# Jiawei-Yang/Denoising-ViT

Measured on AMD Instinct MI355X. Metric: stage-1 images denoised/sec (DINOv2-B/14, 518px, 1k Adam steps), higher is better.
Workload: dtype bf16

## Files before the change

denoising-vit_amd/csrc/dvt_vit.hip:

```cpp
#include <math.h>

#include <type_traits>

#include "../../include/dvt_vit.h"
#include "dvt_common.h"
#include "dvt_ln_row.h"

typedef short bf16x8 __attribute__((ext_vector_type(8)));
typedef short bf16x4 __attribute__((ext_vector_type(4)));
typedef float f32x4 __attribute__((ext_vector_type(4)));
typedef unsigned short bf16_t;

extern int g_f32x3_exact_attention, g_f32x3_unfused;

namespace {

typedef __bf16 hw_bf16x2 __attribute__((ext_vector_type(2)));
typedef float f32x2 __attribute__((ext_vector_type(2)));

__device__ __forceinline__ uint32_t pack2(float a, float b) {
  const hw_bf16x2 v = __builtin_convertvector((f32x2){a, b}, hw_bf16x2);
  return __builtin_bit_cast(uint32_t, v);
}
__device__ __forceinline__ bf16_t f2bf(float f) { return (bf16_t)(pack2(f, 0.f) & 0xffffu); }
// ... 261 lines not shown
        for (int rp = 0; rp < 2; ++rp) {
          const float mine0 = v[rp], mine1 = v[rp + 2];
          const float send = odd ? mine0 : mine1;
          const float recv = __shfl_xor(send, 1, 64);
          const int r = odd ? rp + 2 : rp;
          const uint32_t w = odd ? pack2(recv, mine1) : pack2(mine0, recv);
          const int ncol = odd ? n - 1 : n;
          *reinterpret_cast<uint32_t*>(p.out + (size_t)(mrow + r) * ldo + ncol) = w;
        }
      }
    }
  }
}

template <int EPI>
__global__ __launch_bounds__(256) void gemm_bf16_kernel(GemmBArgs p) {
  __shared__ __attribute__((aligned(16))) char smem[2 * STAGE_BYTES];
  const int tid = threadIdx.x, lane = tid & 63, wave = tid >> 6;
  const int wm = wave >> 1, wn = wave & 1;
  const TileMap tm = map_tile(blockIdx.x, gridDim.x, p.M / GBM, p.N / GBN, p.group);
  const int m0 = tm.m * GBM, n0 = tm.n * GBN;

  f32x4 acc[4][4];
#pragma unroll
  for (int i = 0; i < 4; ++i)
#pragma unroll
    for (int j = 0; j < 4; ++j) acc[i][j] = (f32x4){0.f, 0.f, 0.f, 0.f};

  const int nk = p.K / GBK;
  stage_tile(p.A, p.K, m0, 0, smem, wave, lane);
  stage_tile(p.W, p.K, n0, 0, smem + GBM * GBK * 2, wave, lane);
  __syncthreads();
  for (int kt = 0; kt < nk; ++kt) {
    char* cur = smem + (kt & 1) * STAGE_BYTES;
    char* nxt = smem + ((kt + 1) & 1) * STAGE_BYTES;
    if (kt + 1 < nk) {
      stage_tile(p.A, p.K, m0, (kt + 1) * GBK, nxt, wave, lane);
      stage_tile(p.W, p.K, n0, (kt + 1) * GBK, nxt + GBM * GBK * 2, wave, lane);
    }
    const char* As = cur;
    const char* Bs = cur + GBM * GBK * 2;
#pragma unroll
    for (int ks = 0; ks < 2; ++ks) {
      bf16x8 a[4], b[4];
      const int chunk = ks * 4 + (lane >> 4);
#pragma unroll
      for (int i = 0; i < 4; ++i) a[i] = read_frag(As, wm * 64 + i * 16 + (lane & 15), chunk);
#pragma unroll
      for (int j = 0; j < 4; ++j) b[j] = read_frag(Bs, wn * 64 + j * 16 + (lane & 15), chunk);
#pragma unroll
      for (int i = 0; i < 4; ++i)
#pragma unroll
        for (int j = 0; j < 4; ++j)
          acc[i][j] = __builtin_amdgcn_mfma_f32_16x16x32_bf16(a[i], b[j], acc[i][j], 0, 0, 0);
    }
    __syncthreads();
  }

  gemm_epilogue<EPI>(p, acc, m0, n0, wm, wn, lane);
}

constexpr int EP_LD = 68;
constexpr int EP_WAVE_BYTES = 64 * EP_LD * 4;

template <int NI>
__device__ __forceinline__ void ln_fold(const GemmBArgs& p, f32x4 (&acc)[NI][4], int mrow0, int ncol0, int lane);

struct NextTilePf {
  const bf16_t* src;
  int n;
  unsigned d0, d1;
};
__device__ __forceinline__ void pf_issue(NextTilePf& f) {
  if (f.src == nullptr) return;
  asm volatile("global_load_dword %0, %1, off" : "=v"(f.d0) : "v"(f.src) : "memory");
  if (f.n > 1) asm volatile("global_load_dword %0, %1, off offset:128" : "=v"(f.d1) : "v"(f.src) : "memory");
}
__device__ __forceinline__ void pf_retire(NextTilePf& f) {
  if (f.src == nullptr) return;
  asm volatile("s_waitcnt vmcnt(0)" ::: "memory");
  asm volatile("" ::"v"(f.d0), "v"(f.d1));
}

template <int EPI, int NI = 4>
__device__ __forceinline__ void gemm_epilogue_lds(const GemmBArgs& p, f32x4 (&acc)[NI][4], int m0,
                                                  int n0, int wm, int wn, int wave, int lane,
                                                  char* smem, char* blk0 = nullptr, NextTilePf* pf = nullptr) {
  static_assert(NI == 4 || NI == 2, "64- or 32-row passes");
  constexpr int ROWS = NI * 16;
  const int g = lane >> 4, lc = lane & 15;
  const bool ln = (IS_QKV(EPI) || IS_GELU(EPI) || EPI == EPI_SWIGLU) && p.ln_stats != nullptr;
  float* blk = reinterpret_cast<float*>(blk0 != nullptr ? blk0 : smem + wave * EP_WAVE_BYTES);
  const int nb = n0 + wn * 64;
  if (IS_QKV(EPI) && n0 >= 2 * p.dim) {
    const int mbv = m0 + wm * 64;
    constexpr int TCH = ROWS / 8, FPP = 64 / TCH, NPASS = 64 / FPP;
    const int tc = lane & (TCH - 1), dl = lane / TCH;
    float4 stq[4];
    float csd[NPASS], bfd[NPASS];
    if (ln) {
      const float4* sp = reinterpret_cast<const float4*>(p.ln_stats + mbv + tc * 8);
#pragma unroll
      for (int q = 0; q < 4; ++q) stq[q] = sp[q];
#pragma unroll
      for (int it = 0; it < NPASS; ++it) {
        csd[it] = p.ln_cs[nb + it * FPP + dl];
        bfd[it] = p.bias[nb + it * FPP + dl];
      }
    }
#pragma unroll
    for (int j = 0; j < 4; ++j) {
      const float bias = (p.bias != nullptr && !ln) ? p.bias[nb + j * 16 + lc] : 0.f;
#pragma unroll
      for (int i = 0; i < NI; ++i) {
        const float4 t4 = make_float4(acc[i][j][0] + bias, acc[i][j][1] + bias, acc[i][j][2] + bias, acc[i][j][3] + bias);
        *reinterpret_cast<float4*>(blk + (j * 16 + lc) * EP_LD + i * 16 + 4 * g) = t4;
      }
    }
    asm volatile("s_waitcnt lgkmcnt(0)" ::: "memory");
    const int f0 = nb - 2 * p.dim, hh = f0 >> 6;
    const int trow = mbv + tc * 8, bimg = trow / p.s_pad, s0 = trow - bimg * p.s_pad;
    const bool vst = trow < p.vt_rows;
    bf16_t* const vrow = p.vt + ((size_t)(bimg * p.heads + hh) * 64) * p.s_pad + s0;
#pragma unroll
    for (int it = 0; it < NPASS; ++it) {
      if (pf != nullptr && it == 1) pf_issue(*pf);
      const int d = it * FPP + dl;
      const float4 a = *reinterpret_cast<const float4*>(blk + d * EP_LD + tc * 8);
      const float4 b = *reinterpret_cast<const float4*>(blk + d * EP_LD + tc * 8 + 4);
      float v[8] = {a.x, a.y, a.z, a.w, b.x, b.y, b.z, b.w};
      if (ln) {
        const float cs = csd[it], bf = bfd[it];
#pragma unroll
        for (int q = 0; q < 4; ++q) {
          v[2 * q] = fmaf(stq[q].y, v[2 * q] - stq[q].x * cs, bf);
          v[2 * q + 1] = fmaf(stq[q].w, v[2 * q + 1] - stq[q].z * cs, bf);
        }
      }
      typedef unsigned u32x4v_t __attribute__((ext_vector_type(4)));
      const u32x4v_t hi = {pack2(v[0], v[1]), pack2(v[2], v[3]), pack2(v[4], v[5]), pack2(v[6], v[7])};
      if (vst) *reinterpret_cast<u32x4v_t*>(vrow + (size_t)d * p.s_pad) = hi;
      if constexpr (EPI == EPI_QKV_X3) {
        u32x4v_t lo;
#pragma unroll
        for (int q = 0; q < 4; ++q)
          lo[q] = pack2(v[2 * q] - __uint_as_float(hi[q] << 16), v[2 * q + 1] - __uint_as_float(hi[q] & 0xffff0000u));
        if (vst) *reinterpret_cast<u32x4v_t*>(p.vt_lo + (vrow - p.vt) + (size_t)d * p.s_pad) = lo;
      }
    }
    return;
  }
  float2 st_row = make_float2(0.f, 0.f);
  if (ln && lane < ROWS) st_row = p.ln_stats[m0 + wm * 64 + lane];
  const int c8_ln = (lane & 7) * 8;
  float4 cs0 = make_float4(0.f, 0.f, 0.f, 0.f), cs1 = cs0, bf0 = cs0, bf1 = cs0;
  if (ln && EPI != EPI_RESID && EPI != EPI_EMBED && EPI != EPI_F32 && EPI != EPI_SWIGLU) {
    cs0 = *reinterpret_cast<const float4*>(p.ln_cs + nb + c8_ln);
    cs1 = *reinterpret_cast<const float4*>(p.ln_cs + nb + c8_ln + 4);
    bf0 = *reinterpret_cast<const float4*>(p.bias + nb + c8_ln);
    bf1 = *reinterpret_cast<const float4*>(p.bias + nb + c8_ln + 4);
  }
#ifdef DVT_LAB
  if (!(p.abl & 1))
#endif
#pragma unroll
  for (int j = 0; j < 4; ++j) {
    const float bias = (p.bias != nullptr && !ln) ? p.bias[nb + j * 16 + lc] : 0.f;
#pragma unroll
    for (int i = 0; i < NI; ++i)
#pragma unroll
      for (int r = 0; r < 4; ++r) blk[(i * 16 + 4 * g + r) * EP_LD + j * 16 + lc] = acc[i][j][r] + bias;
  }
  if (ln && lane < ROWS) *reinterpret_cast<float2*>(blk + lane * EP_LD + 64) = st_row;
  asm volatile("s_waitcnt lgkmcnt(0)" ::: "memory");
  const int mb = m0 + wm * 64;
  if constexpr (EPI == EPI_SWIGLU) {
    const int c8 = (lane & 3) * 8, ldo = p.N >> 1;
    const int rsub = ((lane >> 2) & 1) + 8 * ((lane >> 3) & 1) + 2 * (lane >> 4);
    alignas(16) float csg[8], csv[8], bfg[8], bfv[8];
    if (ln) {
#pragma unroll
      for (int q = 0; q < 8; q += 4) {
        *reinterpret_cast<float4*>(csg + q) = *reinterpret_cast<const float4*>(p.ln_cs + nb + c8 + q);
        *reinterpret_cast<float4*>(csv + q) = *reinterpret_cast<const float4*>(p.ln_cs + nb + 32 + c8 + q);
        *reinterpret_cast<float4*>(bfg + q) = *reinterpret_cast<const float4*>(p.bias + nb + c8 + q);
        *reinterpret_cast<float4*>(bfv + q) = *reinterpret_cast<const float4*>(p.bias + nb + 32 + c8 + q);
      }
    }
#pragma unroll 1
    for (int it = 0; it < ROWS / 16; ++it) {
      if (pf != nullptr && it == 1) pf_issue(*pf);
      const int row = it * 16 + rsub;
      alignas(16) float gt[8], vl[8];
#pragma unroll
      for (int q = 0; q < 8; q += 4) {
        *reinterpret_cast<float4*>(gt + q) = *reinterpret_cast<const float4*>(blk + row * EP_LD + c8 + q);
        *reinterpret_cast<float4*>(vl + q) = *reinterpret_cast<const float4*>(blk + row * EP_LD + 32 + c8 + q);
      }
      if (ln) {
        const float2 stv = *reinterpret_cast<const float2*>(blk + row * EP_LD + 64);
#pragma unroll
        for (int q = 0; q < 8; ++q) {
          gt[q] = fmaf(stv.y, gt[q] - stv.x * csg[q], bfg[q]);
          vl[q] = fmaf(stv.y, vl[q] - stv.x * csv[q], bfv[q]);
        }
      }
#pragma unroll
      for (int q = 0; q < 8; ++q) gt[q] = silu_log2(gt[q]) * vl[q];
      typedef unsigned u32x4s_t __attribute__((ext_vector_type(4)));
      const u32x4s_t val = {pack2(gt[0], gt[1]), pack2(gt[2], gt[3]), pack2(gt[4], gt[5]), pack2(gt[6], gt[7])};
      u32x4s_t* dst = reinterpret_cast<u32x4s_t*>(p.out + (size_t)(mb + row) * ldo + (nb >> 1) + c8);
      if (p.nt_store)
        __builtin_nontemporal_store(val, dst);
      else
        *dst = val;
    }
    return;
  }
  if (EPI == EPI_RESID || EPI == EPI_EMBED || EPI == EPI_F32) {
    const int c4 = lc * 4;
    float4 gm = make_float4(1.f, 1.f, 1.f, 1.f);
    if (EPI == EPI_RESID) gm = *reinterpret_cast<const float4*>(p.gamma + nb + c4);
#pragma unroll 4
    for (int it = 0; it < ROWS / 4; ++it) {
      const int row = it * 4 + g;
      if (pf != nullptr && it == ROWS / 8 && EPI == EPI_F32) pf_issue(*pf);
      const float4 v = *reinterpret_cast<const float4*>(blk + row * EP_LD + c4);
      const int t = mb + row;
      float4* px = reinterpret_cast<float4*>(p.x + (size_t)t * p.N + nb + c4);
      if (EPI == EPI_RESID) {
        float4 o = *px;
        o.x += gm.x * v.x;
        o.y += gm.y * v.y;
        o.z += gm.z * v.z;
        o.w += gm.w * v.w;
        *px = o;
      } else if (EPI == EPI_F32) {
        *px = v;
      } else {
        const int sidx = t % p.s_pad;
        float4 o = make_float4(0.f, 0.f, 0.f, 0.f);
        if (sidx < p.n_prefix) {
          o = *reinterpret_cast<const float4*>(p.cls + (size_t)sidx * p.N + nb + c4);
          if (p.pos_has_cls && sidx == 0) {
            const float4 q = *reinterpret_cast<const float4*>(p.pos + nb + c4);
            o = make_float4(o.x + q.x, o.y + q.y, o.z + q.z, o.w + q.w);
          }
        } else if (sidx < p.n_tokens) {
          const float4 q = *reinterpret_cast<const float4*>(
// ... 80 lines not shown
    for (int r = 0; r < 4; ++r) {
      const float2 st = p.ln_stats[mrow0 + i * 16 + 4 * g + r];
#pragma unroll
      for (int j = 0; j < 4; ++j) acc[i][j][r] = st.y * (acc[i][j][r] - st.x * cs[j]);
    }
}

__global__ __launch_bounds__(256) void ln_stats_finalize_kernel(const float2* __restrict__ part, int P, int M, float inv_n,
                                                                float eps, float2* __restrict__ stats) {
  const int m = blockIdx.x * 256 + threadIdx.x;
  if (m >= M) return;
  float s1 = 0.f, s2 = 0.f;
  for (int q = 0; q < P; ++q) {
    const float2 v = part[(size_t)q * M + m];
    s1 += v.x;
    s2 += v.y;
  }
  const float mu = s1 * inv_n;
  const float var = fmaxf(s2 * inv_n - mu * mu, 0.f);
  stats[m] = make_float2(mu, rsqrtf(var + eps));
}

template <int NV = 4>
__global__ __launch_bounds__(256) void ln_cast_stats_kernel(const float* __restrict__ x, bf16_t* __restrict__ xb,
                                                            float2* __restrict__ stats, int rows, int dim, float eps) {
  const int row = blockIdx.x * 4 + (threadIdx.x >> 6), lane = threadIdx.x & 63;
  if (row >= rows) return;
  const float4* xr = reinterpret_cast<const float4*>(x + (size_t)row * dim);
  const int nq = dim >> 2;
  float4 v[NV];
  float sum = 0.f;
#pragma unroll
  for (int i = 0; i < NV; ++i) {
    const int q = lane + 64 * i;
    if (q < nq) {
      v[i] = xr[q];
      sum += v[i].x + v[i].y + v[i].z + v[i].w;
      uint2 pk;
      pk.x = pack2(v[i].x, v[i].y);
      pk.y = pack2(v[i].z, v[i].w);
      reinterpret_cast<uint2*>(xb + (size_t)row * dim)[q] = pk;
    }
  }
  const float mean = wave_sum(sum) / (float)dim;
  float var = 0.f;
#pragma unroll
  for (int i = 0; i < NV; ++i) {
    const int q = lane + 64 * i;
    if (q < nq) {
      const float a = v[i].x - mean, b = v[i].y - mean, c = v[i].z - mean, d = v[i].w - mean;
      var += a * a + b * b + c * c + d * d;
    }
  }
  const float rstd = rsqrtf(wave_sum(var) / (float)dim + eps);
  if (lane == 0) stats[row] = make_float2(mean, rstd);
}

__global__ __launch_bounds__(256) void swiglu_act_kernel(const uint4* __restrict__ h, uint4* __restrict__ hid, long long n8,
                                                         int hq) {
  for (long long q = (long long)blockIdx.x * 256 + threadIdx.x; q < n8; q += (long long)gridDim.x * 256) {
    const long long r = q / hq;
    const int c = (int)(q - r * hq);
    const uint4 gv = h[r * 2 * hq + c], vv = h[r * 2 * hq + hq + c];
    const unsigned gw[4] = {gv.x, gv.y, gv.z, gv.w}, vw[4] = {vv.x, vv.y, vv.z, vv.w};
    unsigned o[4];
#pragma unroll
    for (int i = 0; i < 4; ++i) {
      const float g0 = __uint_as_float(gw[i] << 16), g1 = __uint_as_float(gw[i] & 0xffff0000u);
      const float v0 = __uint_as_float(vw[i] << 16), v1 = __uint_as_float(vw[i] & 0xffff0000u);
      o[i] = pack2(silu_log2(g0) * v0, silu_log2(g1) * v1);
    }
    hid[q] = make_uint4(o[0], o[1], o[2], o[3]);
  }
}

__device__ __forceinline__ float row16_sum(float v) {
  v += __builtin_bit_cast(float, __builtin_amdgcn_update_dpp(0, __builtin_bit_cast(int, v), 0x128, 0xf, 0xf, false));
  v += __builtin_bit_cast(float, __builtin_amdgcn_update_dpp(0, __builtin_bit_cast(int, v), 0x124, 0xf, 0xf, false));
  v += __builtin_bit_cast(float, __builtin_amdgcn_update_dpp(0, __builtin_bit_cast(int, v), 0x122, 0xf, 0xf, false));
  v += __builtin_bit_cast(float, __builtin_amdgcn_update_dpp(0, __builtin_bit_cast(int, v), 0x121, 0xf, 0xf, false));
  return v;
}

__device__ __forceinline__ void gemm_epilogue_resid_sq(const GemmBArgs& p, f32x4 (&acc)[8][4], int mb,
                                                       int nb, int wave, int lane, char* smem, NextTilePf* pf = nullptr) {
  const int g = lane >> 4, lc = lane & 15, c4 = lc * 4;
  float* blk = reinterpret_cast<float*>(smem + wave * EP_WAVE_BYTES);
  const __amdgpu_buffer_rsrc_t xr = __builtin_amdgcn_make_buffer_rsrc(
      p.x + (size_t)mb * p.N + nb, 0, 0x7fffffff, 0x00020000);
  const int loff = (g * p.N + c4) * 4;
  const int rstep = p.N * 16;
  typedef int i32x4_t __attribute__((ext_vector_type(4)));
#define RS_LD(it) __builtin_bit_cast(float4, __builtin_amdgcn_raw_buffer_load_b128(xr, loff, (it) * rstep, 0))
#define RS_ST(it, v) __builtin_amdgcn_raw_buffer_store_b128(__builtin_bit_cast(i32x4_t, v), xr, loff + (it) * rstep, 0, 0)
#define RS_LN(it, o)                                                                                    \
  do {                                                                                                  \
    const int row_ = mb + (it) * 4 + g;                                                                 \
    uint2 pk_;                                                                                          \
    pk_.x = pack2((o).x, (o).y);                                                                        \
    pk_.y = pack2((o).z, (o).w);                                                                        \
    *reinterpret_cast<uint2*>(p.xb + (size_t)row_ * p.N + nb + c4) = pk_;                               \
    float s1_ = ((o).x + (o).y) + ((o).z + (o).w);                                                      \
    float s2_ = ((o).x * (o).x + (o).y * (o).y) + ((o).z * (o).z + (o).w * (o).w);                      \
    s1_ = row16_sum(s1_);                                                                               \
    s2_ = row16_sum(s2_);                                                                               \
    if (lc == 0) p.st_part[(size_t)(nb >> 6) * p.M + row_] = make_float2(s1_, s2_);                     \
  } while (0)
  float4 xl[16], xh[16];
#pragma unroll
  for (int it = 0; it < 16; ++it) xl[it] = RS_LD(it);
  float bias[4];
#pragma unroll
  for (int j = 0; j < 4; ++j) bias[j] = p.bias != nullptr ? p.bias[nb + j * 16 + lc] : 0.f;
  const float4 gm = *reinterpret_cast<const float4*>(p.gamma + nb + c4);
#ifdef DVT_LAB
  if (!(p.abl & 1))
#endif
#pragma unroll
  for (int j = 0; j < 4; ++j)
#pragma unroll
    for (int i = 0; i < 4; ++i)
#pragma unroll
      for (int r = 0; r < 4; ++r) blk[(i * 16 + 4 * g + r) * EP_LD + j * 16 + lc] = acc[i][j][r] + bias[j];
#pragma unroll
  for (int it = 0; it < 16; ++it) xh[it] = RS_LD(16 + it);
  asm volatile("s_waitcnt lgkmcnt(0)" ::: "memory");
#pragma unroll
  for (int it = 0; it < 16; ++it) {
    const float4 v = *reinterpret_cast<const float4*>(blk + (it * 4 + g) * EP_LD + c4);
    float4 o = xl[it];
    o.x += gm.x * v.x;
    o.y += gm.y * v.y;
    o.z += gm.z * v.z;
    o.w += gm.w * v.w;
    RS_ST(it, o);
    if (p.xb != nullptr) RS_LN(it, o);
  }
  asm volatile("s_waitcnt lgkmcnt(0)" ::: "memory");
  if (pf != nullptr) pf_issue(*pf);
#ifdef DVT_LAB
  if (!(p.abl & 1))
#endif
#pragma unroll
  for (int j = 0; j < 4; ++j)
#pragma unroll
    for (int i = 0; i < 4; ++i)
#pragma unroll
      for (int r = 0; r < 4; ++r) blk[(i * 16 + 4 * g + r) * EP_LD + j * 16 + lc] = acc[4 + i][j][r] + bias[j];
  asm volatile("s_waitcnt lgkmcnt(0)" ::: "memory");
#pragma unroll
  for (int it = 0; it < 16; ++it) {
    const float4 v = *reinterpret_cast<const float4*>(blk + (it * 4 + g) * EP_LD + c4);
    float4 o = xh[it];
    o.x += gm.x * v.x;
    o.y += gm.y * v.y;
    o.z += gm.z * v.z;
    o.w += gm.w * v.w;
    RS_ST(16 + it, o);
    if (p.xb != nullptr) RS_LN(16 + it, o);
  }
#undef RS_LD
#undef RS_ST
#undef RS_LN
}

constexpr int G2_BM = 256, G2_STAGE = (G2_BM + GBN) * GBK * 2;

template <int EPI>
__global__ __launch_bounds__(512) __attribute__((amdgpu_waves_per_eu(2, 2))) void gemm_bf16_kernel_pp(GemmBArgs p) {
  __shared__ __attribute__((aligned(16))) char smem[3 * G2_STAGE];
  const int tid = threadIdx.x, lane = tid & 63;
  const int wave = __builtin_amdgcn_readfirstlane(tid >> 6);
  const int wm = wave >> 1, wn = wave & 1;
  const bool group_b = wave >= 4;
  const TileMap tm = map_tile(blockIdx.x, gridDim.x, p.M / G2_BM, p.N / GBN, p.group);
  const int m0 = tm.m * G2_BM, n0 = tm.n * GBN;

  f32x4 acc[4][4];
#pragma unroll
  for (int i = 0; i < 4; ++i)
#pragma unroll
    for (int j = 0; j < 4; ++j) acc[i][j] = (f32x4){0.f, 0.f, 0.f, 0.f};

  const int nk = p.K / GBK;
  const bf16_t* srcA[4];
  const bf16_t* srcW[2];
#pragma unroll
  for (int it = 0; it < 4; ++it) {
    const int s_ = it * 512 + tid, row = s_ >> 3, c = (s_ & 7) ^ (row & 7);
    srcA[it] = p.A + (size_t)(m0 + row) * p.K + c * 8;
    if (it < 2) srcW[it] = p.W + (size_t)(n0 + row) * p.K + c * 8;
  }
  const int ldsw = wave * 1024;
#define PP_ISSUE(kt)                                                                  \
  do {                                                                                \
    char* st_ = smem + ((kt) % 3) * G2_STAGE + ldsw;                                  \
    const int ko_ = (kt) * GBK;                                                       \
    _Pragma("unroll") for (int it = 0; it < 4; ++it)                                  \
        glds16(srcA[it] + ko_, st_ + it * 8192);                                      \
    _Pragma("unroll") for (int it = 0; it < 2; ++it)                                  \
        glds16(srcW[it] + ko_, st_ + G2_BM * GBK * 2 + it * 8192);                    \
  } while (0)
  PP_ISSUE(0);
  if (nk > 1) {
    PP_ISSUE(1);
    asm volatile("s_waitcnt vmcnt(6)" ::: "memory");
  } else {
    asm volatile("s_waitcnt vmcnt(0)" ::: "memory");
  }
  __builtin_amdgcn_s_barrier();
  if (group_b) __builtin_amdgcn_s_barrier();
  const int rowa = wm * 64 + (lane & 15), rowb = wn * 64 + (lane & 15), cg = lane >> 4;
  for (int kt = 0; kt < nk; ++kt) {
    if (kt + 2 < nk) PP_ISSUE(kt + 2);
    const char* As = smem + (kt % 3) * G2_STAGE;
    const char* Bs = As + G2_BM * GBK * 2;
    bf16x8 a0[4], b0[4], a1[4], b1[4];
#pragma unroll
    for (int i = 0; i < 4; ++i) a0[i] = read_frag(As, rowa + i * 16, cg);
#pragma unroll
    for (int j = 0; j < 4; ++j) b0[j] = read_frag(Bs, rowb + j * 16, cg);
#pragma unroll
    for (int i = 0; i < 4; ++i) a1[i] = read_frag(As, rowa + i * 16, 4 + cg);
#pragma unroll
    for (int j = 0; j < 4; ++j) b1[j] = read_frag(Bs, rowb + j * 16, 4 + cg);
    if (kt + 2 < nk)
      asm volatile("s_waitcnt vmcnt(6)" ::: "memory");
    else
      asm volatile("s_waitcnt vmcnt(0)" ::: "memory");
    asm volatile("s_waitcnt lgkmcnt(0)" ::: "memory");
    __builtin_amdgcn_sched_barrier(0);
    __builtin_amdgcn_s_barrier();
    __builtin_amdgcn_sched_barrier(0);
#pragma unroll
    for (int i = 0; i < 4; ++i)
#pragma unroll
      for (int j = 0; j < 4; ++j)
        acc[i][j] = __builtin_amdgcn_mfma_f32_16x16x32_bf16(a0[i], b0[j], acc[i][j], 0, 0, 0);
#pragma unroll
    for (int i = 0; i < 4; ++i)
#pragma unroll
      for (int j = 0; j < 4; ++j)
        acc[i][j] = __builtin_amdgcn_mfma_f32_16x16x32_bf16(a1[i], b1[j], acc[i][j], 0, 0, 0);
    __builtin_amdgcn_sched_barrier(0);
    __builtin_amdgcn_s_barrier();
    __builtin_amdgcn_sched_barrier(0);
  }
#undef PP_ISSUE
  if (!group_b) __builtin_amdgcn_s_barrier();
  __syncthreads();
  gemm_epilogue_lds<EPI>(p, acc, m0, n0, wm, wn, wave, lane, smem);
}

template <int MODE>
struct P8Wait;
template <> struct P8Wait<0> { static constexpr int w1 = 8, w2 = 8, w4 = 8; };
template <> struct P8Wait<1> { static constexpr int w1 = 8, w2 = 8, w4 = 4; };
template <> struct P8Wait<2> { static constexpr int w1 = 2, w2 = 0, w4 = -1; };

template <int N>
__device__ __forceinline__ void wait_vm() {
  if constexpr (N == 8) asm volatile("s_waitcnt vmcnt(8)" ::: "memory");
  else if constexpr (N == 6) asm volatile("s_waitcnt vmcnt(6)" ::: "memory");
  else if constexpr (N == 4) asm volatile("s_waitcnt vmcnt(4)" ::: "memory");
  else if constexpr (N == 2) asm volatile("s_waitcnt vmcnt(2)" ::: "memory");
  else if constexpr (N == 0) asm volatile("s_waitcnt vmcnt(0)" ::: "memory");
}

#define P8_BAR()                         \
  do {                                   \
    __builtin_amdgcn_sched_barrier(0);   \
    __builtin_amdgcn_s_barrier();        \
    __builtin_amdgcn_sched_barrier(0);   \
  } while (0)
#define P8_LGKM0() asm volatile("s_waitcnt lgkmcnt(0)" ::: "memory")
#define P8_MFMA(IB, JB, AF, BF)                                                                   \
  do {                                                                                            \
    __builtin_amdgcn_s_setprio(1);                                                                \
    _Pragma("unroll") for (int ks = 0; ks < 2; ++ks)                                              \
    _Pragma("unroll") for (int i = 0; i < 4; ++i)                                                 \
    _Pragma("unroll") for (int j = 0; j < 2; ++j)                                                 \
        acc[IB + i][JB + j] =                                                                     \
            __builtin_amdgcn_mfma_f32_16x16x32_bf16(AF[i][ks], BF[j][ks], acc[IB + i][JB + j], 0, 0, 0); \
    __builtin_amdgcn_s_setprio(0);                                                                \
  } while (0)

template <int MODE>
struct P8BWait;
template <> struct P8BWait<0> { static constexpr int w1 = 8, w2 = 8, w3 = 8, w4 = 8; };
template <> struct P8BWait<1> { static constexpr int w1 = 8, w2 = 8, w3 = 6, w4 = 4; };
template <> struct P8BWait<2> { static constexpr int w1 = 2, w2 = 0, w3 = -1, w4 = -1; };
template <> struct P8BWait<3> { static constexpr int w1 = -1, w2 = -1, w3 = 8, w4 = 8; };
template <> struct P8BWait<4> { static constexpr int w1 = 4, w2 = 4, w3 = -1, w4 = -1; };

typedef __attribute__((address_space(3))) void* lds_ptr_t;

#define P8_LANE_SETUP()                                                                                                  \
  int voA[2], voB[2];                                                                                                    \
  _Pragma("unroll") for (int it = 0; it < 2; ++it) {                                                                     \
    const int s_ = it * 512 + tid, r = s_ >> 3, c = (s_ & 7) ^ (r & 7);                                                  \
    voA[it] = (((r >> 6) * 128 + (r & 63)) * p.lda + c * 8) * 2;                                                         \
    voB[it] = (((r >> 5) * 64 + (r & 31)) * p.ldw + c * 8) * 2;                                                          \
  }                                                                                                                      \
  const int hA = 64 * p.lda * 2, hB = 32 * p.ldw * 2;                     \
  constexpr int OFF_A0 = 0, OFF_A1 = 16384, OFF_B0 = 32768, OFF_B1 = 49152, BUF = 65536;                                 \
  char* const ldsw = smem + wave * 1024;                                                                                 \
  const int cg = lane >> 4;                                                                                              \
  const int ra = wm * 64 + (lane & 15), rb = wn * 32 + (lane & 15);                                                      \
  const int oa0 = ra * 128 + (((0 + cg) ^ (ra & 7)) << 4), oa1 = ra * 128 + (((4 + cg) ^ (ra & 7)) << 4);                \
  const int ob0 = rb * 128 + (((0 + cg) ^ (rb & 7)) << 4), ob1 = rb * 128 + (((4 + cg) ^ (rb & 7)) << 4);                \
  int oa0q = oa0 + 65536, oa1q = oa1 + 65536, ob0q = ob0 + 65536, ob1q = ob1 + 65536;                                    \
  asm volatile("" : "+v"(oa0q), "+v"(oa1q), "+v"(ob0q), "+v"(ob1q))
#define P8_RSRC(ptr, len) __builtin_amdgcn_make_buffer_rsrc((void*)(ptr), 0, (len), 0x00020000)
#define P8_STAGE_RS(RS, X, H, kt, off)                                                                                   \
  do {                                                                                                                   \
    const int so_ = (kt) * (GBK * 2) + (H) * h##X;                                                                       \
    __builtin_amdgcn_raw_ptr_buffer_load_lds(RS, (lds_ptr_t)(ldsw + (off)), 16, vo##X[0], so_, 0, P8_AUX_##X);           \
    __builtin_amdgcn_raw_ptr_buffer_load_lds(RS, (lds_ptr_t)(ldsw + (off) + 8192), 16, vo##X[1], so_, 0, P8_AUX_##X);    \
  } while (0)
#define P8_STAGE(X, H, kt, off) P8_STAGE_RS(rs##X, X, H, kt, off)
#define P8_RD(base, off) (*reinterpret_cast<const bf16x8*>((base) + (off)))
#define P8B_TILE(MODE, PAR, t, BC, BX)                                                            \
  do {                                                                                            \
    constexpr int bo_ = (PAR) * BUF, bn_ = bo_ ^ BUF;                                             \
    constexpr bool st12_ = MODE == 0 || MODE == 1 || MODE == 3, st34_ = MODE == 0 || MODE == 3;   \
    const int ra0_ = (PAR) ? oa0q : oa0, ra1_ = (PAR) ? oa1q : oa1;     \
    const int rb0_ = (PAR) ? ob0q : ob0, rb1_ = (PAR) ? ob1q : ob1;               \
    const int rn0_ = (PAR) ? ob0 : ob0q, rn1_ = (PAR) ? ob1 : ob1q;     \
                                                                                          \
    _Pragma("unroll") for (int i = 0; i < 4; ++i) {                                               \
      a[i][0] = P8_RD(smem + OFF_A0 + i * 2048, ra0_);                                            \
      a[i][1] = P8_RD(smem + OFF_A0 + i * 2048, ra1_);                                            \
    }                                                                                             \
    if (st12_) P8_STAGE(B, 1, (t) + 1, bn_ + OFF_B1);                                             \
    if (MODE == 4) P8_STAGE_RS(rsBn, B, 0, 0, OFF_B0);                                            \
    wait_vm<P8BWait<MODE>::w1>();                                                                 \
    P8_BAR();                                                                                     \
    P8_LGKM0();                                                                                   \
    P8_MFMA(0, 0, a, BC);                                                                         \
    P8_BAR();                                                                                     \
                                                                                          \
    _Pragma("unroll") for (int j = 0; j < 2; ++j) {                                               \
      BX[j][0] = P8_RD(smem + OFF_B1 + j * 2048, rb0_);                                           \
      BX[j][1] = P8_RD(smem + OFF_B1 + j * 2048, rb1_);                                           \
    }                                                                                             \
    if (st12_) P8_STAGE(A, 1, (t) + 1, bn_ + OFF_A1);                                             \
    if (MODE == 4) P8_STAGE_RS(rsAn, A, 0, 0, OFF_A0);                                            \
    wait_vm<P8BWait<MODE>::w2>();                                                                 \
    P8_BAR();                                                                                     \
    P8_LGKM0();                                                                                   \
    P8_MFMA(0, 2, a, BX);                                                                         \
    P8_BAR();                                                                                     \
                                                                                          \
    _Pragma("unroll") for (int i = 0; i < 4; ++i) {                                               \
      a[i][0] = P8_RD(smem + OFF_A1 + i * 2048, ra0_);                                            \
      a[i][1] = P8_RD(smem + OFF_A1 + i * 2048, ra1_);                                            \
    }                                                                                             \
    if (st34_) P8_STAGE(B, 0, (t) + 2, bo_ + OFF_B0);                                             \
    if (MODE == 4) P8_STAGE_RS(rsBn, B, 1, 0, OFF_B1);                                            \
    wait_vm<P8BWait<MODE>::w3>();                                                                 \
    P8_BAR();                                                                                     \
    P8_LGKM0();                                                                                   \
    P8_MFMA(4, 2, a, BX);                                                                         \
    P8_BAR();                                                                                     \
                          \
    if (MODE != 2 && MODE != 4) {                                                                 \
      _Pragma("unroll") for (int j = 0; j < 2; ++j) {                                             \
        BX[j][0] = P8_RD(smem + OFF_B0 + j * 2048, rn0_);                                         \
        BX[j][1] = P8_RD(smem + OFF_B0 + j * 2048, rn1_);                                         \
      }                                                                                           \
    }                                                                                             \
    if (st34_) P8_STAGE(A, 0, (t) + 2, bo_ + OFF_A0);                                             \
    if (MODE == 4) P8_STAGE_RS(rsAn, A, 1, 0, OFF_A1);                                            \
    wait_vm<P8BWait<MODE>::w4>();                                                                 \
    P8_BAR();                                                                                     \
    P8_MFMA(4, 0, a, BC);                                                                         \
    P8_BAR();                                                                                     \
  } while (0)

template <int EPI, bool STAMP = false, int AUX = 0>
__global__ __launch_bounds__(512) __attribute__((amdgpu_waves_per_eu(2, 2))) void gemm_bf16_kernel_8p(GemmBArgs p) {
  constexpr int P8_AUX_A = (AUX & 1) ? 2 : 0, P8_AUX_B = (AUX & 2) ? 2 : 0;
  __shared__ __attribute__((aligned(16))) char smem[8 * EP_WAVE_BYTES];
  unsigned long long ts_[5] = {0, 0, 0, 0, 0};
  if constexpr (STAMP) ts_[0] = __builtin_amdgcn_s_memrealtime();
  if (p.stagger_ticks > 0 && blockIdx.x < 256) {
    const unsigned h_ = ((unsigned)blockIdx.x * 2654435761u) >> 16;
    const unsigned long long wait_ = ((unsigned long long)p.stagger_ticks * h_) >> 16;
    const unsigned long long t0_ = __builtin_amdgcn_s_memrealtime();
    while (__builtin_amdgcn_s_memrealtime() - t0_ < wait_) __builtin_amdgcn_s_sleep(16);
  }
  const int tid = threadIdx.x, lane = tid & 63;
  const int wave = __builtin_amdgcn_readfirstlane(tid >> 6);
  const int wm = wave >> 2, wn = wave & 3;
  const TileMap tm = map_tile_fast(p, blockIdx.x, gridDim.x, p.M >> 8, p.N >> 8);
  const int m0 = tm.m * 256, n0 = tm.n * 256;

  f32x4 acc[8][4];
#pragma unroll
  for (int i = 0; i < 8; ++i)
#pragma unroll
    for (int j = 0; j < 4; ++j) acc[i][j] = (f32x4){0.f, 0.f, 0.f, 0.f};

  const int nk = p.K / GBK;
  P8_LANE_SETUP();
  const __amdgpu_buffer_rsrc_t rsA = P8_RSRC(p.A + (size_t)m0 * p.lda, 0x7fffffff);
  const __amdgpu_buffer_rsrc_t rsB = P8_RSRC(p.W + (size_t)n0 * p.ldw, 0x7fffffff);
  const __amdgpu_buffer_rsrc_t rsAn = rsA, rsBn = rsB;

  unsigned ts_setup_ = 0, ts_issued_ = 0;
  if constexpr (STAMP) {
    asm volatile("" : "+v"(voA[0]), "+v"(voB[0]), "+v"(oa0q));
    ts_setup_ = (unsigned)__builtin_amdgcn_s_memrealtime();
  }
  P8_STAGE(B, 0, 0, OFF_B0);
  P8_STAGE(A, 0, 0, OFF_A0);
  P8_STAGE(B, 1, 0, OFF_B1);
  P8_STAGE(A, 1, 0, OFF_A1);
  P8_STAGE(B, 0, 1, BUF + OFF_B0);
  P8_STAGE(A, 0, 1, BUF + OFF_A0);
  if constexpr (STAMP) ts_issued_ = (unsigned)__builtin_amdgcn_s_memrealtime();
  wait_vm<8>();
  P8_BAR();
  if (wm == 1) P8_BAR();

  bf16x8 a[4][2], be[2][2], bo[2][2];
#pragma unroll
  for (int j = 0; j < 2; ++j) {
    be[j][0] = P8_RD(smem + OFF_B0 + j * 2048, ob0);
    be[j][1] = P8_RD(smem + OFF_B0 + j * 2048, ob1);
  }
  if constexpr (STAMP) ts_[1] = __builtin_amdgcn_s_memrealtime();
  int t = 0;
  for (; t < nk - 2; t += 2) {
    P8B_TILE(0, 0, t, be, bo);
    P8B_TILE(0, 1, t + 1, bo, be);
  }
  P8B_TILE(1, 0, t, be, bo);
  P8B_TILE(2, 1, t + 1, bo, be);
  if (wm == 0) P8_BAR();
  __syncthreads();
  if constexpr (STAMP) ts_[2] = __builtin_amdgcn_s_memrealtime();
  NextTilePf pf_{nullptr, p.pf_next, 0u, 0u};
  if (p.pf_next > 0 && (int)blockIdx.x + 256 < (int)gridDim.x) {
    const TileMap tn = map_tile_fast(p, blockIdx.x + 256, gridDim.x, p.M >> 8, p.N >> 8);
    pf_.src = tid < 256 ? p.A + (size_t)(tn.m * 256 + tid) * p.lda : p.W + (size_t)(tn.n * 256 + tid - 256) * p.ldw;
  }
  if constexpr (EPI == EPI_RESID) {
    gemm_epilogue_resid_sq(p, acc, m0 + wm * 128, n0 + wn * 64, wave, lane, smem, &pf_);
  } else {
    f32x4(&lo)[4][4] = *reinterpret_cast<f32x4(*)[4][4]>(&acc[0]);
    f32x4(&hi)[4][4] = *reinterpret_cast<f32x4(*)[4][4]>(&acc[4]);
    gemm_epilogue_lds<EPI>(p, lo, m0 + wm * 128, n0 + wn * 64, 0, 0, wave, lane, smem);
    asm volatile("s_waitcnt lgkmcnt(0)" ::: "memory");
    gemm_epilogue_lds<EPI>(p, hi, m0 + wm * 128 + 64, n0 + wn * 64, 0, 0, wave, lane, smem, nullptr, &pf_);
  }
  pf_retire(pf_);
  if constexpr (STAMP) {
    ts_[3] = __builtin_amdgcn_s_memrealtime();
    asm volatile("s_waitcnt vmcnt(0)" ::: "memory");
    ts_[4] = __builtin_amdgcn_s_memrealtime();
    if (p.dbg != nullptr && tid == 0) {
      unsigned* d_ = p.dbg + (size_t)blockIdx.x * 8;
#pragma unroll
      for (int i = 0; i < 5; ++i) d_[i] = (unsigned)ts_[i];
      d_[5] = __builtin_amdgcn_s_getreg((31 << 11) | 4);
      d_[6] = __builtin_amdgcn_s_getreg((31 << 11) | 20);
      d_[7] = ((ts_setup_ - (unsigned)ts_[0]) & 0xffffu) | ((ts_issued_ - (unsigned)ts_[0]) << 16);
    }
  }
}

#ifdef DVT_LAB
#include "lab/dvt_vit_gemm8t.inc"
#endif
#undef P8B_TILE
#undef P8_STAGE
#undef P8_STAGE_RS
#undef P8_RSRC
#undef P8_RD
#undef P8_LANE_SETUP

#ifdef DVT_LAB
typedef const __attribute__((address_space(4))) GemmBArgs* kernarg_ptr_t;

__device__ __forceinline__ TileMap map_tile_id(int id, int mt, int nt, int group, int mblock) {
  const int per_group = group * mt;
  int g = id / per_group;
  const int full = nt / group;
  int width = group;
  if (g >= full) {
    g = full;
    width = nt - full * group;
  }
  const int rem = id - g * per_group;
  TileMap t;
  if (mblock <= 1) {
    t.m = rem / width;
    t.n = g * group + rem % width;
  } else {
    const int per_block = mblock * width;
    const int mbk = rem / per_block, r2 = rem - mbk * per_block;
    const int left = mt - mbk * mblock, hb = left < mblock ? left : mblock;
    t.n = g * group + r2 / hb;
    t.m = mbk * mblock + r2 % hb;
  }
  return t;
}


#include "lab/dvt_vit_gemm4w.inc"
#include "lab/dvt_vit_gemm8p_lab.inc"
#include "lab/dvt_vit_lab.inc"
#endif

int g_vit_group_bytes = 4800 * 1024;
int g_vit_mblock = 0;
int g_vit_nt_store = 0;
int g_vit_fuse_ln = 1;
int g_vit_attn_mask = 15;
int g_vit_stagger_pct = 0;
int g_vit_attn_log2q = 1;
constexpr float ATT_Q_PRESCALE = 0.125f * 1.4426950408889634f;
int g_vit_pf_next = 0;
constexpr int ATT_L2_VAR = 559;
#ifdef DVT_LAB
int g_vit_tpw = 0;
int g_vit_attn_l2_mask = ATT_L2_VAR;
int g_vit_epi_abl = 0;
int g_vit_attn_variant = 2;
int g_vit_abl4w = 0;
int g_vit_8p_build = 0;
unsigned* g_vit_dbg = nullptr;
int g_vit_w4_grid = 0;
#endif

template <int EPI>
int launch_gemm(const GemmBArgs& a0, hipStream_t s) {
// ... 1686 lines not shown
```

denoising-vit_amd/csrc/lab/dvt_vit_gemm8t.inc:

```
template <int EPI>
__global__ __launch_bounds__(512) __attribute__((amdgpu_waves_per_eu(2, 2))) void gemm_bf16_kernel_8t(GemmBArgs p) {
  constexpr int P8_AUX_A = 0, P8_AUX_B = 0;
  __shared__ __attribute__((aligned(16))) char smem[8 * EP_WAVE_BYTES];
  static_assert(EPI == EPI_BIAS || EPI == EPI_QKV || EPI == EPI_GELU, "epilogues with 32-row passes");
  const int tid = threadIdx.x, lane = tid & 63;
  const int wave = __builtin_amdgcn_readfirstlane(tid >> 6);
  const int wm = wave >> 2, wn = wave & 3;
  const int mt = p.M / 256, nt = p.N / 256, total = mt * nt;
  int v = ((int)blockIdx.x >> 8) * p.tpw * 256 + ((int)blockIdx.x & 255);
  int left = p.tpw;
  if (v >= total) return;
  const int nk = p.K / GBK;
  TileMap tm = map_tile(v, total, mt, nt, p.group, p.mblock);
  int m0 = tm.m * 256, n0 = tm.n * 256;
  __amdgpu_buffer_rsrc_t rsA = P8_RSRC(p.A + (size_t)m0 * p.lda, 0x7fffffff);
  __amdgpu_buffer_rsrc_t rsB = P8_RSRC(p.W + (size_t)n0 * p.ldw, 0x7fffffff);
  char* const stg = smem + 65536 + wave * 9216;
  {
    P8_LANE_SETUP();
    P8_STAGE(B, 0, 0, OFF_B0);
    P8_STAGE(A, 0, 0, OFF_A0);
    P8_STAGE(B, 1, 0, OFF_B1);
    P8_STAGE(A, 1, 0, OFF_A1);
  }
  bool first = true;
  f32x4 acc[8][4];
  for (;;) {
    int tid = threadIdx.x;
    asm volatile("" : "+v"(tid));
    const int lane = tid & 63;
    P8_LANE_SETUP();
    P8_BAR();
    P8_STAGE(B, 0, 1, BUF + OFF_B0);
    P8_STAGE(A, 0, 1, BUF + OFF_A0);
    if (first) asm volatile("s_waitcnt vmcnt(4)" ::: "memory");
    else asm volatile("s_waitcnt vmcnt(20)" ::: "memory");
    first = false;
    P8_BAR();
    if (wm == 1) P8_BAR();
    const int vn = v + 256;
    --left;
    const bool more = left > 0 && vn < total;
    const TileMap tn = map_tile(more ? vn : v, total, mt, nt, p.group, p.mblock);
    const int m0n = tn.m * 256, n0n = tn.n * 256;
    const __amdgpu_buffer_rsrc_t rsAn = P8_RSRC(p.A + (size_t)m0n * p.lda, more ? 0x7fffffff : 0);
    const __amdgpu_buffer_rsrc_t rsBn = P8_RSRC(p.W + (size_t)n0n * p.ldw, more ? 0x7fffffff : 0);
    bf16x8 a[4][2], be[2][2], bo[2][2];
#pragma unroll
    for (int i = 0; i < 8; ++i)
#pragma unroll
      for (int j = 0; j < 4; ++j) acc[i][j] = (f32x4){0.f, 0.f, 0.f, 0.f};
#pragma unroll
    for (int j = 0; j < 2; ++j) {
      be[j][0] = P8_RD(smem + OFF_B0 + j * 2048, ob0);
      be[j][1] = P8_RD(smem + OFF_B0 + j * 2048, ob1);
    }
    P8B_TILE(3, 0, 0, be, bo);
    P8B_TILE(0, 1, 1, bo, be);
    for (int t = 2; t < nk - 2; t += 2) {
      P8B_TILE(0, 0, t, be, bo);
      P8B_TILE(0, 1, t + 1, bo, be);
    }
    P8B_TILE(1, 0, nk - 2, be, bo);
    P8B_TILE(4, 1, nk - 1, bo, be);
    if (wm == 0) P8_BAR();
    P8_BAR();
#pragma unroll
    for (int q = 0; q < 4; ++q) {
      f32x4(&part)[2][4] = *reinterpret_cast<f32x4(*)[2][4]>(&acc[2 * q]);
      gemm_epilogue_lds<EPI, 2>(p, part, m0 + wm * 128 + q * 32, n0 + wn * 64, 0, 0, wave, lane, smem, stg);
      asm volatile("s_waitcnt lgkmcnt(0)" ::: "memory");
    }
    if (!more) break;
    v = vn;
    m0 = m0n;
    n0 = n0n;
    rsA = rsAn;
    rsB = rsBn;
  }
}
```

Measured before the change: 3.016.

## Swap MFMA operands for row-major accumulators in RESID/GELU/EMBED/F32 epilogues

```diff
diff --git a/denoising-vit_amd/csrc/dvt_vit.hip b/denoising-vit_amd/csrc/dvt_vit.hip
--- a/denoising-vit_amd/csrc/dvt_vit.hip
+++ b/denoising-vit_amd/csrc/dvt_vit.hip
@@ -367,11 +367,12 @@
   asm volatile("" ::"v"(f.d0), "v"(f.d1));
 }
 
-template <int EPI, int NI = 4>
+template <int EPI, int NI = 4, bool RM = false>
 __device__ __forceinline__ void gemm_epilogue_lds(const GemmBArgs& p, f32x4 (&acc)[NI][4], int m0,
                                                   int n0, int wm, int wn, int wave, int lane,
                                                   char* smem, char* blk0 = nullptr, NextTilePf* pf = nullptr) {
   static_assert(NI == 4 || NI == 2, "64- or 32-row passes");
+  static_assert(!RM || EPI == EPI_EMBED || EPI == EPI_F32, "row-major accumulators: the fp32 outputs");
   constexpr int ROWS = NI * 16;
   const int g = lane >> 4, lc = lane & 15;
   const bool ln = (IS_QKV(EPI) || IS_GELU(EPI) || EPI == EPI_SWIGLU) && p.ln_stats != nullptr;
@@ -450,6 +451,12 @@
 #endif
 #pragma unroll
   for (int j = 0; j < 4; ++j) {
+    if constexpr (RM) {
+      const f32x4 bias4 = p.bias != nullptr ? *reinterpret_cast<const f32x4*>(p.bias + nb + j * 16 + 4 * g) : (f32x4){0.f, 0.f, 0.f, 0.f};
+#pragma unroll
+      for (int i = 0; i < NI; ++i) *reinterpret_cast<f32x4*>(blk + (i * 16 + lc) * EP_LD + j * 16 + 4 * g) = acc[i][j] + bias4;
+      continue;
+    }
     const float bias = (p.bias != nullptr && !ln) ? p.bias[nb + j * 16 + lc] : 0.f;
 #pragma unroll
     for (int i = 0; i < NI; ++i)
@@ -696,6 +703,7 @@
   return v;
 }
 
+template <bool RM = false>
 __device__ __forceinline__ void gemm_epilogue_resid_sq(const GemmBArgs& p, f32x4 (&acc)[8][4], int mb,
                                                        int nb, int wave, int lane, char* smem, NextTilePf* pf = nullptr) {
   const int g = lane >> 4, lc = lane & 15, c4 = lc * 4;
@@ -725,23 +733,32 @@
   for (int it = 0; it < 16; ++it) xl[it] = RS_LD(it);
   float bias[4];
 #pragma unroll
-  for (int j = 0; j < 4; ++j) bias[j] = p.bias != nullptr ? p.bias[nb + j * 16 + lc] : 0.f;
+  for (int j = 0; j < 4; ++j) bias[j] = (!RM && p.bias != nullptr) ? p.bias[nb + j * 16 + lc] : 0.f;
+  float4 brb = make_float4(0.f, 0.f, 0.f, 0.f);
+  if (RM && p.bias != nullptr) brb = *reinterpret_cast<const float4*>(p.bias + nb + c4);
   const float4 gm = *reinterpret_cast<const float4*>(p.gamma + nb + c4);
 #ifdef DVT_LAB
   if (!(p.abl & 1))
 #endif
 #pragma unroll
-  for (int j = 0; j < 4; ++j)
-#pragma unroll
-    for (int i = 0; i < 4; ++i)
-#pragma unroll
-      for (int r = 0; r < 4; ++r) blk[(i * 16 + 4 * g + r) * EP_LD + j * 16 + lc] = acc[i][j][r] + bias[j];
+  for (int j = 0; j < 4; ++j) {
+#pragma unroll
+    for (int i = 0; i < 4; ++i) {
+      if constexpr (RM) {
+        *reinterpret_cast<f32x4*>(blk + (i * 16 + lc) * EP_LD + j * 16 + 4 * g) = acc[i][j];
+      } else {
+#pragma unroll
+        for (int r = 0; r < 4; ++r) blk[(i * 16 + 4 * g + r) * EP_LD + j * 16 + lc] = acc[i][j][r] + bias[j];
+      }
+    }
+  }
 #pragma unroll
   for (int it = 0; it < 16; ++it) xh[it] = RS_LD(16 + it);
   asm volatile("s_waitcnt lgkmcnt(0)" ::: "memory");
 #pragma unroll
   for (int it = 0; it < 16; ++it) {
-    const float4 v = *reinterpret_cast<const float4*>(blk + (it * 4 + g) * EP_LD + c4);
+    float4 v = *reinterpret_cast<const float4*>(blk + (it * 4 + g) * EP_LD + c4);
+    if constexpr (RM) v = make_float4(v.x + brb.x, v.y + brb.y, v.z + brb.z, v.w + brb.w);
     float4 o = xl[it];
     o.x += gm.x * v.x;
     o.y += gm.y * v.y;
@@ -758,13 +775,19 @@
 #pragma unroll
   for (int j = 0; j < 4; ++j)
 #pragma unroll
-    for (int i = 0; i < 4; ++i)
-#pragma unroll
-      for (int r = 0; r < 4; ++r) blk[(i * 16 + 4 * g + r) * EP_LD + j * 16 + lc] = acc[4 + i][j][r] + bias[j];
+    for (int i = 0; i < 4; ++i) {
+      if constexpr (RM) {
+        *reinterpret_cast<f32x4*>(blk + (i * 16 + lc) * EP_LD + j * 16 + 4 * g) = acc[4 + i][j];
+      } else {
+#pragma unroll
+        for (int r = 0; r < 4; ++r) blk[(i * 16 + 4 * g + r) * EP_LD + j * 16 + lc] = acc[4 + i][j][r] + bias[j];
+      }
+    }
   asm volatile("s_waitcnt lgkmcnt(0)" ::: "memory");
 #pragma unroll
   for (int it = 0; it < 16; ++it) {
-    const float4 v = *reinterpret_cast<const float4*>(blk + (it * 4 + g) * EP_LD + c4);
+    float4 v = *reinterpret_cast<const float4*>(blk + (it * 4 + g) * EP_LD + c4);
+    if constexpr (RM) v = make_float4(v.x + brb.x, v.y + brb.y, v.z + brb.z, v.w + brb.w);
     float4 o = xh[it];
     o.x += gm.x * v.x;
     o.y += gm.y * v.y;
@@ -776,6 +799,77 @@
 #undef RS_LD
 #undef RS_ST
 #undef RS_LN
+}
+
+
+constexpr int EPB_LD = 144;
+__device__ __forceinline__ void gemm_epilogue_rm_gelu(const GemmBArgs& p, f32x4 (&acc)[8][4], int mb, int nb, int wave, int lane,
+                                                      char* smem, NextTilePf* pf = nullptr) {
+  const int g = lane >> 4, lc = lane & 15, c4 = 4 * g;
+  const bool ln = p.ln_stats != nullptr;
+  char* blk = smem + wave * EP_WAVE_BYTES;
+  char* const wr = blk + lc * EPB_LD + g * 8;
+  const char* const rd = blk + (lane >> 3) * EPB_LD + (lane & 7) * 16;
+  bf16_t* const orow = p.out + (size_t)(mb + (lane >> 3)) * p.N + nb + (lane & 7) * 8;
+  typedef unsigned u32x4_t __attribute__((ext_vector_type(4)));
+  float4 cs[4], bf[4];
+#pragma unroll
+  for (int j = 0; j < 4; ++j) {
+    cs[j] = bf[j] = make_float4(0.f, 0.f, 0.f, 0.f);
+    if (p.bias != nullptr) bf[j] = *reinterpret_cast<const float4*>(p.bias + nb + j * 16 + c4);
+    if (ln) cs[j] = *reinterpret_cast<const float4*>(p.ln_cs + nb + j * 16 + c4);
+  }
+  float2 st[4];
+#pragma unroll
+  for (int i = 0; i < 4; ++i) st[i] = ln ? p.ln_stats[mb + i * 16 + lc] : make_float2(0.f, 1.f);
+#pragma unroll
+  for (int h = 0; h < 2; ++h) {
+#pragma unroll
+    for (int i4 = 0; i4 < 4; ++i4) {
+      const int i = h * 4 + i4;
+      const float mu = st[i4].x, rs = st[i4].y;
+#pragma unroll
+      for (int j = 0; j < 4; ++j) {
+        float v0 = acc[i][j][0], v1 = acc[i][j][1], v2 = acc[i][j][2], v3 = acc[i][j][3];
+        if (ln) {
+          v0 = fmaf(rs, v0 - mu * cs[j].x, bf[j].x);
+          v1 = fmaf(rs, v1 - mu * cs[j].y, bf[j].y);
+          v2 = fmaf(rs, v2 - mu * cs[j].z, bf[j].z);
+          v3 = fmaf(rs, v3 - mu * cs[j].w, bf[j].w);
+        } else {
+          v0 += bf[j].x;
+          v1 += bf[j].y;
+          v2 += bf[j].z;
+          v3 += bf[j].w;
+        }
+        gelu_erf_pair(v0, v1);
+        gelu_erf_pair(v2, v3);
+        uint2 pk;
+        pk.x = pack2(v0, v1);
+        pk.y = pack2(v2, v3);
+#ifdef DVT_LAB
+        if (!(p.abl & 1))
+#endif
+        *reinterpret_cast<uint2*>(wr + i4 * 16 * EPB_LD + j * 32) = pk;
+      }
+    }
+    asm volatile("s_waitcnt lgkmcnt(0)" ::: "memory");
+    if (h == 0 && ln) {
+#pragma unroll
+      for (int i = 0; i < 4; ++i) st[i] = p.ln_stats[mb + 64 + i * 16 + lc];
+    }
+#pragma unroll
+    for (int it = 0; it < 8; ++it) {
+      if (pf != nullptr && h == 1 && it == 1) pf_issue(*pf);
+      const u32x4_t val = *reinterpret_cast<const u32x4_t*>(rd + it * 8 * EPB_LD);
+      u32x4_t* dst = reinterpret_cast<u32x4_t*>(orow + (size_t)(h * 64 + it * 8) * p.N);
+      if (p.nt_store)
+        __builtin_nontemporal_store(val, dst);
+      else
+        *dst = val;
+    }
+    asm volatile("s_waitcnt lgkmcnt(0)" ::: "memory");
+  }
 }
 
 constexpr int G2_BM = 256, G2_STAGE = (G2_BM + GBN) * GBK * 2;
@@ -888,16 +982,20 @@
     __builtin_amdgcn_sched_barrier(0);   \
   } while (0)
 #define P8_LGKM0() asm volatile("s_waitcnt lgkmcnt(0)" ::: "memory")
-#define P8_MFMA(IB, JB, AF, BF)                                                                   \
+#define P8_MFMA_O(IB, JB, AF, BF, SWAP)                                                           \
   do {                                                                                            \
     __builtin_amdgcn_s_setprio(1);                                                                \
     _Pragma("unroll") for (int ks = 0; ks < 2; ++ks)                                              \
     _Pragma("unroll") for (int i = 0; i < 4; ++i)                                                 \
     _Pragma("unroll") for (int j = 0; j < 2; ++j)                                                 \
-        acc[IB + i][JB + j] =                                                                     \
-            __builtin_amdgcn_mfma_f32_16x16x32_bf16(AF[i][ks], BF[j][ks], acc[IB + i][JB + j], 0, 0, 0); \
+        acc[IB + i][JB + j] = (SWAP)                                                              \
+            ? __builtin_amdgcn_mfma_f32_16x16x32_bf16(BF[j][ks], AF[i][ks], acc[IB + i][JB + j], 0, 0, 0)  \
+            : __builtin_amdgcn_mfma_f32_16x16x32_bf16(AF[i][ks], BF[j][ks], acc[IB + i][JB + j], 0, 0, 0); \
     __builtin_amdgcn_s_setprio(0);                                                                \
   } while (0)
+#define P8_MFMA(IB, JB, AF, BF) P8_MFMA_O(IB, JB, AF, BF, false)
+template <int EPI>
+struct P8Swap { static constexpr bool v = EPI == EPI_RESID || EPI == EPI_GELU || EPI == EPI_EMBED || EPI == EPI_F32; };
 
 template <int MODE>
 struct P8BWait;
@@ -951,7 +1049,7 @@
     wait_vm<P8BWait<MODE>::w1>();                                                                 \
     P8_BAR();                                                                                     \
     P8_LGKM0();                                                                                   \
-    P8_MFMA(0, 0, a, BC);                                                                         \
+    P8_MFMA_O(0, 0, a, BC, P8_SWAP);                                                              \
     P8_BAR();                                                                                     \
                                                                                           \
     _Pragma("unroll") for (int j = 0; j < 2; ++j) {                                               \
@@ -963,7 +1061,7 @@
     wait_vm<P8BWait<MODE>::w2>();                                                                 \
     P8_BAR();                                                                                     \
     P8_LGKM0();                                                                                   \
-    P8_MFMA(0, 2, a, BX);                                                                         \
+    P8_MFMA_O(0, 2, a, BX, P8_SWAP);                                                              \
     P8_BAR();                                                                                     \
                                                                                           \
     _Pragma("unroll") for (int i = 0; i < 4; ++i) {                                               \
@@ -975,7 +1073,7 @@
     wait_vm<P8BWait<MODE>::w3>();                                                                 \
     P8_BAR();                                                                                     \
     P8_LGKM0();                                                                                   \
-    P8_MFMA(4, 2, a, BX);                                                                         \
+    P8_MFMA_O(4, 2, a, BX, P8_SWAP);                                                              \
     P8_BAR();                                                                                     \
                           \
     if (MODE != 2 && MODE != 4) {                                                                 \
@@ -988,13 +1086,14 @@
     if (MODE == 4) P8_STAGE_RS(rsAn, A, 1, 0, OFF_A1);                                            \
     wait_vm<P8BWait<MODE>::w4>();                                                                 \
     P8_BAR();                                                                                     \
-    P8_MFMA(4, 0, a, BC);                                                                         \
+    P8_MFMA_O(4, 0, a, BC, P8_SWAP);                                                              \
     P8_BAR();                                                                                     \
   } while (0)
 
 template <int EPI, bool STAMP = false, int AUX = 0>
 __global__ __launch_bounds__(512) __attribute__((amdgpu_waves_per_eu(2, 2))) void gemm_bf16_kernel_8p(GemmBArgs p) {
   constexpr int P8_AUX_A = (AUX & 1) ? 2 : 0, P8_AUX_B = (AUX & 2) ? 2 : 0;
+  constexpr bool P8_SWAP = P8Swap<EPI>::v;
   __shared__ __attribute__((aligned(16))) char smem[8 * EP_WAVE_BYTES];
   unsigned long long ts_[5] = {0, 0, 0, 0, 0};
   if constexpr (STAMP) ts_[0] = __builtin_amdgcn_s_memrealtime();
@@ -1061,13 +1160,16 @@
     pf_.src = tid < 256 ? p.A + (size_t)(tn.m * 256 + tid) * p.lda : p.W + (size_t)(tn.n * 256 + tid - 256) * p.ldw;
   }
   if constexpr (EPI == EPI_RESID) {
-    gemm_epilogue_resid_sq(p, acc, m0 + wm * 128, n0 + wn * 64, wave, lane, smem, &pf_);
+    gemm_epilogue_resid_sq<P8_SWAP>(p, acc, m0 + wm * 128, n0 + wn * 64, wave, lane, smem, &pf_);
+  } else if constexpr (EPI == EPI_GELU) {
+    gemm_epilogue_rm_gelu(p, acc, m0 + wm * 128, n0 + wn * 64, wave, lane, smem, &pf_);
   } else {
+    static_assert(!P8_SWAP || EPI == EPI_EMBED || EPI == EPI_F32, "the other LDS-staged epilogues take column-layout accumulators");
     f32x4(&lo)[4][4] = *reinterpret_cast<f32x4(*)[4][4]>(&acc[0]);
     f32x4(&hi)[4][4] = *reinterpret_cast<f32x4(*)[4][4]>(&acc[4]);
-    gemm_epilogue_lds<EPI>(p, lo, m0 + wm * 128, n0 + wn * 64, 0, 0, wave, lane, smem);
+    gemm_epilogue_lds<EPI, 4, P8_SWAP>(p, lo, m0 + wm * 128, n0 + wn * 64, 0, 0, wave, lane, smem);
     asm volatile("s_waitcnt lgkmcnt(0)" ::: "memory");
-    gemm_epilogue_lds<EPI>(p, hi, m0 + wm * 128 + 64, n0 + wn * 64, 0, 0, wave, lane, smem, nullptr, &pf_);
+    gemm_epilogue_lds<EPI, 4, P8_SWAP>(p, hi, m0 + wm * 128 + 64, n0 + wn * 64, 0, 0, wave, lane, smem, nullptr, &pf_);
   }
   pf_retire(pf_);
   if constexpr (STAMP) {
diff --git a/denoising-vit_amd/csrc/lab/dvt_vit_gemm8t.inc b/denoising-vit_amd/csrc/lab/dvt_vit_gemm8t.inc
--- a/denoising-vit_amd/csrc/lab/dvt_vit_gemm8t.inc
+++ b/denoising-vit_amd/csrc/lab/dvt_vit_gemm8t.inc
@@ -1,6 +1,7 @@
 template <int EPI>
 __global__ __launch_bounds__(512) __attribute__((amdgpu_waves_per_eu(2, 2))) void gemm_bf16_kernel_8t(GemmBArgs p) {
   constexpr int P8_AUX_A = 0, P8_AUX_B = 0;
+  constexpr bool P8_SWAP = false;
   __shared__ __attribute__((aligned(16))) char smem[8 * EP_WAVE_BYTES];
   static_assert(EPI == EPI_BIAS || EPI == EPI_QKV || EPI == EPI_GELU, "epilogues with 32-row passes");
   const int tid = threadIdx.x, lane = tid & 63;
```

After: 3.019 (median of 6 runs). About the same (+0.1%).
